# bioinfo-ut/PhenotypeSeeker

Measured on AMD Instinct MI355X. Metric: k-mer x sample chi2 cells/sec, higher is better.
Workload: dtype u64 popcount + f64; 1 GPU; synthetic 256 x 5.0-Mbp FASTA, binary phenotype, k=13; n_samples=256, k=13, rows_per_gpu=22950458, words_per_row_stored=4, survivors=1736, survivors_all_slabs=1736, device= (gfx950:sramecc+:xnack-), rows_global=22950458, collectives=none

## Files before the change

### phenotypeseeker_amd/csrc/assoc_scan.hip

```cpp
#include "chi2_launch.h"

namespace {

__device__ __forceinline__ double chi2_exact(double A, double B, double C, double D)
{
    const double w_pheno = A + B, wo_pheno = C + D, w_kmer = A + C, wo_kmer = B + D;
    const double total = w_pheno + wo_pheno;
    const double e0 = (w_pheno * w_kmer) / total, e1 = (w_pheno * wo_kmer) / total;
    const double e2 = (wo_pheno * w_kmer) / total, e3 = (wo_pheno * wo_kmer) / total;
    double stat = 0.0, d;
    d = A - e0; stat += (d * d) / e0;
    d = B - e1; stat += (d * d) / e1;
    d = C - e2; stat += (d * d) / e2;
    d = D - e3; stat += (d * d) / e3;
    return stat;
}

__device__ __forceinline__ bool chi2_keep(const ScanCuts &K, double A, double B, double C, double D, double &stat, double &p, bool valid = true)
{
    stat = chi2_exact(A, B, C, D);
    p = exp(-0.5 * stat);
    return valid && ((K.omit_B && p < K.pcut) || (p < K.pcut_bonf));
}

// ... 331 lines not shown
        b += stride;
    }
    publish_segment_once(X.s.sink);
}

template <int CPR>
__global__ __launch_bounds__(CX_IDX_THREADS) void chi2_scan_kernel_cx_side_idx(const CxSideIdxArgs X)
{
    const ScanCuts &K = X.s.cut;
    const ScanSink &S = X.s.sink;
    stamp_scan_start(S);
    if (blockIdx.x == 0) publish_unowned_segments(S);
    const int lane = threadIdx.x & 63;
    const uint64_t e0 = X.run_len[0], e1 = e0 + X.run_len[1], e2 = e1 + X.run_len[2], T = e2 + X.run_len[3];
    const uint32_t seg = blockIdx.x & (SC_NSEG - 1);
    for (uint64_t t0 = (uint64_t)blockIdx.x * CX_IDX_THREADS; t0 < T; t0 += (uint64_t)gridDim.x * CX_IDX_THREADS) {
        const uint64_t t = t0 + threadIdx.x;
        const bool live = t < T;
        uint32_t a = 0, c = 0, row = 0;
        if (live) {
            const uint64_t pos = t < e0 ? X.run_begin[0] + t : t < e1 ? X.run_begin[1] + (t - e0) : t < e2 ? X.run_begin[2] + (t - e1) : X.run_begin[3] + (t - e2);
            const uint64_t j = X.idx[pos];
            u32x4 x[CPR];
#pragma unroll
            for (int g = 0; g < CPR; g++) x[g] = PSK_CX_SIDE_NT ? __builtin_nontemporal_load(&X.s.ov[j * CPR + g]) : X.s.ov[j * CPR + g];
            row = X.s.ov_row[j];
#pragma unroll
            for (int g = 0; g < CPR; g++) {
                const uint64_t xa = ((uint64_t)x[g].y << 32) | x[g].x, xb = ((uint64_t)x[g].w << 32) | x[g].z;
                a += __popcll(xa & X.s.m1[2 * g]) + __popcll(xb & X.s.m1[2 * g + 1]);
                c += __popcll(xa & X.s.m0[2 * g]) + __popcll(xb & X.s.m0[2 * g + 1]);
            }
        }
        const int n_w = (int)(a + c);
        const int n_wo = (K.n1 - (int)a) + (K.n0 - (int)c);
        const bool freq_ok = live && !(n_w < K.min_samples || n_wo < 2 || n_w > K.max_samples);
        const double A = (double)a, B = (double)(K.n1 - (int)a), C = (double)c, D = (double)(K.n0 - (int)c);
        double stat = 0.0, p = 1.0;
        bool keep = false;
        if (freq_ok && chi2_pretest(A, B, C, D, K.thr)) keep = chi2_keep(K, A, B, C, D, stat, p);
        const uint64_t keepers = __ballot(keep);
        if (keepers) {
            uint32_t base = 0;
            if (lane == 0) base = atomicAdd(&S.counter[seg * SC_CNT_STRIDE], (uint32_t)__popcll(keepers));
            base = __builtin_amdgcn_readfirstlane(base);
            if (keep) {
                const uint32_t idx = base + (uint32_t)__popcll(keepers & ((1ull << lane) - 1ull));
                chi2_store(S, (uint64_t)seg * S.seg_cap + (idx < S.seg_cap ? idx : S.seg_cap - 1), row, stat, p, n_w);
            }
        }
    }
    publish_segment_once(S);
}

__global__ __launch_bounds__(SC_FIN_THREADS) void chi2w_finalize_kernel(const ScanArgs P)
{
    __shared__ uint32_t scan_lds[SC_FIN_THREADS / 64];
    __shared__ uint32_t s_out;
    __shared__ double2 s_tab[SC_FIN_BLK * 128];
    const uint32_t seg = blockIdx.x;
    const uint32_t c = P.sink.counter[seg * SC_CNT_STRIDE];
    const uint64_t base = (uint64_t)seg * P.sink.seg_cap;
    if (threadIdx.x == 0) s_out = 0;
    __syncthreads();
    for (uint32_t s0 = 0; s0 < c; s0 += SC_FIN_THREADS) {
        const uint32_t i = s0 + threadIdx.x;
        const bool valid = i < c;
// ... 96 lines not shown
```

### phenotypeseeker_amd/csrc/chi2_driver.hip

```cpp
#include "chi2_launch.h"

#include <cmath>
#include <sched.h>

namespace {

int pick_chi2_mode(psk_ctx *ctx, bool weighted, double pcut, double pcut_bonf, int omit_B, int *mode)
{
    double expect = pcut_bonf;
    if (omit_B && pcut > expect) expect = pcut;
    *mode = weighted ? 1 : ctx->dense_hint >= 0 ? (ctx->dense_hint ? 2 : 0) : expect > 1e-3 ? 2 : 0;
    return weighted ? PSK_OK : env_choice(ctx, "PSK_CHI2_MODE", {0, 2}, mode);
}

uint64_t cx_side_grid_cap(const psk_ctx *ctx) { return (uint64_t)(ctx->n_cu > 0 ? ctx->n_cu : 256) * (ctx->grid_mult ? ctx->grid_mult : PSK_CX_SIDE_GRID_MULT); }
uint64_t cx_pc_grid_cap(const psk_ctx *ctx) { return (uint64_t)(ctx->n_cu > 0 ? ctx->n_cu : 256) * (ctx->grid_mult ? ctx->grid_mult : PSK_CX_PC_GRID_MULT); }

int run_chi2(psk_ctx *ctx, const Chi2Launch &L, int reps, double *ms_total, double *ms_each = nullptr)
{
    *ms_total = 0;
    for (int r = 0; r < reps; r++) {
        launch_chi2_any(ctx, L, {ctx->ev0, ctx->ev1});
        PSK_HIP(ctx, hipGetLastError());
        PSK_HIP(ctx, hipStreamSynchronize(ctx->stream));
// ... 100 lines not shown
    CL.form = Chi2Form::Dense;
    ctx->last_form = (int)CL.form;
    PSK_TRY(pick_chi2_mode(ctx, L.weighted, a.cut.pcut, a.cut.pcut_bonf, a.cut.omit_B, &CL.mode));
    CL.grid = sh.grid;
    return setup_results(ctx, a, CL.grid, group_lanes(a), sh.unroll, set, sh.threads);
}

int chi2_scan_launch(psk_ctx *ctx, const int8_t *pheno, const double *weights, int min_samples, int max_samples,
                     double pvalue_cutoff, int omit_B, uint64_t n_kmers_global, bool keep_results)
{
    if (!ctx) return PSK_EINVAL;
    if (ctx->n_in_flight >= 2) return psk_fail(ctx, PSK_ESTATE, "two scans are in flight (psk_scan_end first)");
    if (!ctx->have_presence) return psk_fail(ctx, PSK_ESTATE, "no presence matrix (psk_build_presence first)");
    if (!pheno) return psk_fail(ctx, PSK_EINVAL, "null phenotype vector");
    if (n_kmers_global == 0) n_kmers_global = ctx->n_kmers ? ctx->n_kmers : 1;
    int wait_by_stamps = 1;
    PSK_TRY(env_choice(ctx, "PSK_SCAN_WAIT", {0, 1}, &wait_by_stamps));
    PSK_HIP(ctx, hipSetDevice(ctx->device));
    const int N = ctx->n_samples, wpr = mask_words(ctx);
    const size_t n_mask = 2 * (size_t)wpr, n_w = 2 * (size_t)wpr * 64;
    const size_t stage_bytes = (n_mask + n_w) * 8;
    int set = 0;
    PSK_TRY(pick_result_set(ctx, &set, keep_results));
    if (2 * stage_bytes > ctx->scan_pinned_cap) {
        if (ctx->n_in_flight) PSK_HIP(ctx, hipStreamSynchronize(ctx->stream));
        if (ctx->scan_pinned) (void)hipHostFree(ctx->scan_pinned);
        ctx->scan_pinned = nullptr;
        ctx->scan_pinned_cap = 0;
        PSK_HIP(ctx, hipHostMalloc(&ctx->scan_pinned, 2 * stage_bytes, hipHostMallocDefault));
        ctx->scan_pinned_cap = 2 * stage_bytes;
    }
    uint64_t *m1 = reinterpret_cast<uint64_t *>(static_cast<uint8_t *>(ctx->scan_pinned) + set * stage_bytes), *m0 = m1 + wpr;
// ... 22 lines not shown
    ctx->last.min_samples = min_samples;
    ctx->last.max_samples = max_samples;
    ctx->last.pvalue_cutoff = pvalue_cutoff;
    ctx->last.omit_B = omit_B ? 1 : 0;
    ctx->last.n_kmers_global = n_kmers_global;
    ctx->last.n1 = n1; ctx->last.n0 = n0; ctx->last.W1 = W1; ctx->last.W0 = W0;
    Chi2Launch CL;
    PSK_TRY(fill_chi2_args(ctx, CL, set, true));
    ctx->last_scan_kind = 1;
    if (ctx->n_kmers) {
        ScanSlot &sl = ctx->slot[set];
        const bool stamped = wait_by_stamps == 1 && !weights && !ctx->exports_async;
        launch_chi2_any(ctx, CL, stamped ? TimedBy{} : TimedBy{sl.ev0, sl.ev1});
        PSK_HIP(ctx, hipGetLastError());
        sl.stamped = stamped;
        sl.in_flight = true;
        ctx->n_in_flight++;
    } else {
        ctx->n_pass = 0;
        ctx->seg_counts.assign(SC_NSEG, 0);
        ctx->res_set = set;
        ctx->results_valid = true;
    }
    return PSK_OK;
}

int rescan(psk_ctx *ctx, int reps, double *mean_ms, double *ms_each)
{
    if (!ctx) return PSK_EINVAL;
    if (ctx->n_in_flight) return psk_fail(ctx, PSK_ESTATE, "a scan is in flight (psk_scan_end first)");
    if (!ctx->have_presence || !ctx->last.valid || ctx->last_scan_kind != 1)
        return psk_fail(ctx, PSK_ESTATE, "no chi2 scan to repeat");
    if (reps < 1) return psk_fail(ctx, PSK_EINVAL, "reps must be >= 1");
    PSK_HIP(ctx, hipSetDevice(ctx->device));
    int set = 0;
    PSK_TRY(pick_result_set(ctx, &set));
    Chi2Launch CL;
    PSK_TRY(fill_chi2_args(ctx, CL, set, false));
    double ms = 0;
    PSK_TRY(run_chi2(ctx, CL, reps, &ms, ms_each));
    ctx->last_scan_ms = ms / reps;
    PSK_TRY(fetch_counts(ctx, set));
    if (mean_ms) *mean_ms = ms / reps;
    return PSK_OK;
}

int wait_stamps(psk_ctx *ctx, int set)
{
    using clk = std::chrono::steady_clock;
    constexpr auto QUERY_EVERY = std::chrono::microseconds(20), YIELD_AFTER = std::chrono::microseconds(50);
    constexpr auto WAIT_LIMIT = std::chrono::seconds(30);
    const volatile uint64_t *counts = scan_stamp_words(ctx, set), *clocks = counts + STAMP_NSEG;
    const uint32_t seq = (uint32_t)ctx->slot[set].seq;
    int nc = 0, nk = 0;
    auto all_here = [&] {
        nc = stamp_counts_missing(counts, seq, nc);
        if (nc == STAMP_NSEG) nk = stamp_clocks_missing(clocks, seq, nk);
        return nc == STAMP_NSEG && nk == STAMP_CLOCKS;
    };
    if (!all_here()) {
        const clk::time_point t0 = clk::now();
        clk::time_point next_query = t0 + QUERY_EVERY;
        for (;;) {
            __builtin_ia32_pause();
            if (all_here()) break;
            const clk::time_point now = clk::now();
            if (now >= next_query) {
                const hipError_t e = hipStreamQuery(ctx->stream);
                if (e == hipSuccess) {
                    if (all_here()) break;
                    return psk_fail(ctx, PSK_ESTATE, "scan ended without publishing (segment %d of scan %u)", nc < STAMP_NSEG ? nc : nk, seq);
                }
                if (e != hipErrorNotReady) return psk_fail(ctx, PSK_EHIP, "hipStreamQuery failed while scan %u was awaited: %s", seq, hipGetErrorString(e));
                (void)hipGetLastError();
                if (now - t0 > WAIT_LIMIT) return psk_fail(ctx, PSK_ESTATE, "scan %u has not published its counts after 30 s", seq);
                next_query = clk::now() + QUERY_EVERY;
            }
            if (now - t0 > YIELD_AFTER) sched_yield();
        }
    }
    ctx->last_scan_ms = (double)stamp_scan_ticks(clocks) / ctx->wall_clock_khz;
    return PSK_OK;
}

}

extern "C" int psk_chi2_scan_begin(psk_ctx *ctx, const int8_t *pheno, const double *weights, int min_samples,
                                   int max_samples, double pvalue_cutoff, int omit_B, uint64_t n_kmers_global)
{
    return chi2_scan_launch(ctx, pheno, weights, min_samples, max_samples, pvalue_cutoff, omit_B, n_kmers_global, true);
}

extern "C" int psk_scan_end(psk_ctx *ctx, uint64_t *n_pass)
{
    if (!ctx) return PSK_EINVAL;
    if (ctx->n_in_flight) {
        PSK_HIP(ctx, hipSetDevice(ctx->device));
        int set = ctx->slot[0].in_flight ? 0 : 1;
        if (ctx->slot[0].in_flight && ctx->slot[1].in_flight && ctx->slot[1].seq < ctx->slot[0].seq) set = 1;
        ScanSlot &sl = ctx->slot[set];
        if (sl.stamped) {
            const int rc = wait_stamps(ctx, set);
            sl.in_flight = false;
            ctx->n_in_flight--;
            PSK_TRY(rc);
        } else {
            PSK_HIP(ctx, hipEventSynchronize(sl.ev1));
            sl.in_flight = false;
            ctx->n_in_flight--;
            float ms = 0;
            PSK_HIP(ctx, hipEventElapsedTime(&ms, sl.ev0, sl.ev1));
            ctx->last_scan_ms = ms;
        }
        PSK_TRY(fetch_counts(ctx, set));
        ctx->dense_hint = ctx->n_pass * 1000 > ctx->n_kmers ? 1 : 0;
    }
    if (n_pass) *n_pass = ctx->n_pass;
    return PSK_OK;
}

extern "C" int psk_chi2_scan(psk_ctx *ctx, const int8_t *pheno, const double *weights, int min_samples,
                             int max_samples, double pvalue_cutoff, int omit_B, uint64_t n_kmers_global,
                             uint64_t *n_pass)
{
    if (ctx && ctx->n_in_flight) return psk_fail(ctx, PSK_ESTATE, "a scan is in flight (psk_scan_end first)");
    PSK_TRY(chi2_scan_launch(ctx, pheno, weights, min_samples, max_samples, pvalue_cutoff, omit_B, n_kmers_global, false));
    return psk_scan_end(ctx, n_pass);
}

// ... 94 lines not shown
```

### phenotypeseeker_amd/csrc/psk_internal.h

```cpp
#pragma once
#include <hip/hip_runtime.h>

#include <cstdarg>
#include <cstdint>
#include <cstdio>
#include <cstdlib>
#include <cstring>
#include <chrono>
#include <functional>
#include <initializer_list>
#include <string>
#include <thread>
#include <utility>
#include <vector>

#include "../../include/psk.h"
#include "chi2_plan.h"

struct DevBuf {
    void *p = nullptr;
    size_t cap = 0;
    bool borrowed = false;
    template <class T> T *as() const { return reinterpret_cast<T *>(p); }
};
// ... 62 lines not shown
    double *res_stat, *res_p, *res_mx, *res_my;
    int32_t *res_nw;
    uint32_t *counter;
    uint32_t *final_counts;
    uint64_t *host_counts;
    uint32_t seg_cap;
    uint32_t seq;
};

struct ScanSlot {
    DevBuf res;
    ScanSink sink = {};
    bool sink_valid = false;
    hipEvent_t ev0 = nullptr, ev1 = nullptr;
    bool stamped = false;
    hipEvent_t ev_ended = nullptr;
    hipEvent_t ev_export = nullptr;
    bool export_pending = false;
    bool in_flight = false;
    uint64_t seq = 0;
    uint64_t seg_cap = 0;
};

struct psk_ctx {
    int device = 0;
    hipStream_t stream = nullptr;
    hipEvent_t ev0 = nullptr, ev1 = nullptr;
    ScanSlot slot[2];
    int res_set = 0;
    bool results_valid = false;
// ... 56 lines not shown
    bool cx_valid = false;
    uint64_t cx_n_ov = 0;
    bool cx_last_plan = false, cx_last_skipped = false, cx_last_filtered = false;
    uint64_t cx_last_rows_feasible = 0;
    uint32_t cx_last_class_mask = 0;
    int last_form = -1;
    CxPlan cx_plan;

    DevBuf mask1, phe, res_count, res_sorted;
    DevBuf lut;
    bool lut_valid = false;
    bool lut6_valid = false;
    uint64_t n_pass = 0;
    uint64_t res_seg_cap = 0;
    std::vector<uint32_t> seg_counts;
    int last_scan_kind = 0;
    int dense_hint = -1;
    double last_scan_ms = 0;
    ScanParams last;

    void *comm = nullptr;
};

int psk_fail(psk_ctx *ctx, int code, const char *fmt, ...);
std::string psk_error_text(psk_ctx *ctx);
void psk_set_error_text(psk_ctx *ctx, const std::string &text);
void psk_forget_lane_slices(psk_ctx *ctx);

#define PSK_HIP(ctx, call)                                                                            \
    do {                                                                                              \
// ... 172 lines not shown
```

### phenotypeseeker_amd/csrc/scan_common.h

```cpp
#pragma once
#include "dev_utils.h"
#include "psk_internal.h"
#include "chi2_plan.h"
#include "scan_stamps.h"

#include <hip/hip_ext.h>
#include <type_traits>

#ifndef PSK_SC_UNROLL
#define PSK_SC_UNROLL 4
#endif
#ifndef PSK_SC_GRID_MULT
#define PSK_SC_GRID_MULT 16
#endif
#ifndef PSK_SC_NT
#define PSK_SC_NT 1
#endif
constexpr int SC_THREADS = 256;
#ifndef PSK_LUT_THREADS
#define PSK_LUT_THREADS 1024
#endif
constexpr int SC_LUT_THREADS = PSK_LUT_THREADS;
constexpr size_t SC_LUT_MAX_BYTES = 132 * 1024;
constexpr int SC_UNROLL = PSK_SC_UNROLL;
// ... 32 lines not shown
    const uint32_t seg = blockIdx.x & (SC_NSEG - 1);
    const uint32_t idx = atomicAdd(&S.counter[seg * SC_CNT_STRIDE], 1u);
    return (uint64_t)seg * S.seg_cap + (idx < S.seg_cap ? idx : S.seg_cap - 1);
}

__device__ __forceinline__ void append_candidate(const ScanSink &S, uint64_t row, int n_w)
{
    const uint64_t idx = reserve_slot(S);
    S.res_row[idx] = row;
    S.res_nw[idx] = n_w;
}

__device__ __forceinline__ void stamp_store(uint64_t *p, uint64_t v) { __hip_atomic_store(p, v, __ATOMIC_RELAXED, __HIP_MEMORY_SCOPE_SYSTEM); }
__device__ __forceinline__ void stamp_clock(const ScanSink &S, int slot) { stamp_store(S.host_counts + STAMP_NSEG + slot, stamp_clock_word(S.seq, (uint64_t)wall_clock64())); }
__device__ __forceinline__ void stamp_count(const ScanSink &S, uint32_t seg, uint32_t c) { stamp_store(S.host_counts + seg, stamp_count_word(S.seq, c)); }
__device__ __forceinline__ void stamp_segment(const ScanSink &S, uint32_t seg, uint32_t c)
{
    stamp_clock(S, (int)seg);
    stamp_count(S, seg, c);
}
__device__ __forceinline__ void stamp_scan_start(const ScanSink &S)
{
    if (blockIdx.x == 0 && threadIdx.x == 0) stamp_clock(S, STAMP_START);
}

__device__ __forceinline__ void publish_segment(const ScanSink &S)
{
    __syncthreads();
    if (threadIdx.x != 0) return;
    const uint32_t seg = blockIdx.x & (SC_NSEG - 1);
    const uint32_t n_blocks = (gridDim.x - seg + SC_NSEG - 1) / SC_NSEG;
    uint32_t *slot = &S.counter[seg * SC_CNT_STRIDE];
    if (atomicAdd(slot + 1, 1u) == n_blocks - 1) {
        const uint32_t c = atomicExch(slot, 0u);
// ... 9 lines not shown
    if (threadIdx.x != 0) return;
    const uint32_t seg = blockIdx.x & (SC_NSEG - 1);
    const uint32_t n_blocks = (gridDim.x - seg + SC_NSEG - 1) / SC_NSEG;
    unsigned long long *slot = reinterpret_cast<unsigned long long *>(&S.counter[seg * SC_CNT_STRIDE]);
    const unsigned long long old = atomicAdd(slot, 1ull << 32);
    if ((uint32_t)(old >> 32) == n_blocks - 1) {
        const uint32_t c = (uint32_t)old;
        *slot = 0ull;
        S.final_counts[seg] = c;
        stamp_segment(S, seg, c);
    }
}

__device__ __forceinline__ void publish_unowned_segments(const ScanSink &S)
{
    for (uint32_t seg = gridDim.x + threadIdx.x; seg < (uint32_t)SC_NSEG; seg += blockDim.x) {
        S.final_counts[seg] = 0;
        stamp_segment(S, seg, 0);
    }
}

int mask_words(const psk_ctx *ctx);
int group_lanes(const ScanArgs &a);
uint64_t scan_grid_cap(const psk_ctx *ctx);
dim3 scan_grid(const psk_ctx *ctx, uint64_t M, int G, int unroll, bool lut = false);
uint64_t result_seg_cap(dim3 grid, uint64_t rows_per_block);
int bind_results(psk_ctx *ctx, ScanSink &s, uint64_t seg_cap, int set);
int setup_results_rows(psk_ctx *ctx, ScanSink &s, dim3 grid, uint64_t rows_per_block, int set);
int setup_results(psk_ctx *ctx, ScanArgs &a, dim3 grid, int G, int unroll, int set, int threads = SC_THREADS);
int pick_result_set(psk_ctx *ctx, int *set_out, bool keep_results = false);
int fetch_counts(psk_ctx *ctx, int set);
const volatile uint64_t *scan_stamp_words(const psk_ctx *ctx, int set);
struct ScanShape {
    dim3 grid;
    int unroll, threads;
};
int setup_table_scan(psk_ctx *ctx, ScanArgs &a, const double *tab, int nm, double s0, double s1, double s2, bool build, ScanShape *sh);

constexpr int sc_rpw(int G) { return G == 0 ? 128 : 64 / G; }
constexpr int sc_lanes(int G) { return G == 0 ? 1 : G; }
template <bool HALF>
__device__ __forceinline__ const u32x4 *sc_row_ptr(const ScanArgs &P, uint64_t r)
{
    if (HALF) return reinterpret_cast<const u32x4 *>(reinterpret_cast<const uint2 *>(P.bits) + r);
    return P.bits + r * (uint64_t)P.cpr;
}
template <bool HALF>
// ... 301 lines not shown
```

### phenotypeseeker_amd/csrc/scan_results.hip

```cpp
#include "scan_common.h"

#include <algorithm>
#include <numeric>

int mask_words(const psk_ctx *ctx) { return (ctx->wpr + 1) & ~1; }

int group_lanes(const ScanArgs &a)
{
    if (a.half) return 0;
    int G = 1;
    while (G < a.cpr && G < 64) G <<= 1;
    return G;
}

uint64_t result_seg_cap(dim3 grid, uint64_t rows_per_block) { return result_seg_cap((uint64_t)grid.x, rows_per_block); }

int bind_results(psk_ctx *ctx, ScanSink &s, uint64_t seg_cap, int set)
{
    if (seg_cap >= (1ull << 32)) return psk_fail(ctx, PSK_ERANGE, "result segment too large");
    ScanSlot &sl = ctx->slot[set];
    if (!sl.sink_valid || sl.sink.seg_cap != (uint32_t)seg_cap) {
        sl.sink_valid = false;
        const uint64_t cap = seg_cap * SC_NSEG;
        DevBuf &rb = sl.res;
        PSK_TRY(dev_reserve(ctx, rb, cap * 44 + 64));
        uint8_t *b = rb.as<uint8_t>();
        ScanSink &a = sl.sink;
        a.res_row = reinterpret_cast<uint64_t *>(b);
        a.res_stat = reinterpret_cast<double *>(b + cap * 8);
        a.res_p = reinterpret_cast<double *>(b + cap * 16);
        a.res_mx = reinterpret_cast<double *>(b + cap * 24);
        a.res_my = reinterpret_cast<double *>(b + cap * 32);
        a.res_nw = reinterpret_cast<int32_t *>(b + cap * 40);
        if (!ctx->res_count.p) {
            PSK_TRY(dev_reserve(ctx, ctx->res_count, (SC_NSEG * SC_CNT_STRIDE + 2 * SC_NSEG) * 4));
            PSK_HIP(ctx, hipMemsetAsync(ctx->res_count.p, 0, (SC_NSEG * SC_CNT_STRIDE + 2 * SC_NSEG) * 4, ctx->stream));
        }
        if (!ctx->cnt_pinned) {
            void *blk = nullptr, *hc = nullptr;
            PSK_HIP(ctx, hipHostMalloc(&blk, 2 * STAMP_SET_WORDS * 8, hipHostMallocCoherent));
            memset(blk, 0, 2 * STAMP_SET_WORDS * 8);
            if (hipHostGetDevicePointer(&hc, blk, 0) != hipSuccess) {
                (void)hipHostFree(blk);
                return psk_fail(ctx, PSK_EHIP, "hipHostGetDevicePointer failed for the scans' stamp block");
            }
            int khz = 0;
            if (hipDeviceGetAttribute(&khz, hipDeviceAttributeWallClockRate, ctx->device) != hipSuccess || khz <= 0) {
                (void)hipHostFree(blk);
                return psk_fail(ctx, PSK_EHIP, "the device reports no wall clock rate");
            }
            ctx->wall_clock_khz = khz;
            ctx->cnt_pinned = blk;
            ctx->cnt_pinned_dev = static_cast<uint64_t *>(hc);
        }
        a.counter = ctx->res_count.as<uint32_t>();
        a.final_counts = a.counter + SC_NSEG * SC_CNT_STRIDE + set * SC_NSEG;
        a.host_counts = ctx->cnt_pinned_dev + set * STAMP_SET_WORDS;
        a.seg_cap = (uint32_t)seg_cap;
        sl.sink_valid = true;
    }
    sl.stamped = false;
    sl.seq = ctx->scan_seq++;
    s = sl.sink;
    s.seq = (uint32_t)sl.seq;
    sl.seg_cap = seg_cap;
    if (set == ctx->res_set) ctx->results_valid = false;
    return PSK_OK;
}

const volatile uint64_t *scan_stamp_words(const psk_ctx *ctx, int set)
{
    return static_cast<const volatile uint64_t *>(ctx->cnt_pinned) + set * STAMP_SET_WORDS;
}

int setup_results_rows(psk_ctx *ctx, ScanSink &s, dim3 grid, uint64_t rows_per_block, int set)
{
    return bind_results(ctx, s, result_seg_cap(grid, rows_per_block), set);
}

int setup_results(psk_ctx *ctx, ScanArgs &a, dim3 grid, int G, int unroll, int set, int threads)
{
// ... 12 lines not shown
    ctx->seg_counts.assign(SC_NSEG, 0);
    uint64_t tot = 0;
    for (int s = 0; s < SC_NSEG; s++) {
        const uint64_t w = stamp_load(raw + s);
        if (stamp_word_seq(w) != seq)
            return psk_fail(ctx, PSK_ESTATE, "result segment %d carries the count of scan %u, not of scan %u", s, stamp_word_seq(w), seq);
        const uint32_t c = stamp_word_count(w);
        if (c > seg_cap) return psk_fail(ctx, PSK_ERANGE, "result segment %d overflowed (%u > %llu)", s, c, (unsigned long long)seg_cap);
        ctx->seg_counts[s] = c;
        tot += c;
    }
    ctx->n_pass = tot;
    ctx->res_set = set;
    ctx->res_seg_cap = seg_cap;
    ctx->results_valid = true;
    return PSK_OK;
}

uint64_t scan_grid_cap(const psk_ctx *ctx) { return (uint64_t)(ctx->n_cu > 0 ? ctx->n_cu : 256) * (ctx->grid_mult ? ctx->grid_mult : PSK_SC_GRID_MULT); }

dim3 scan_grid(const psk_ctx *ctx, uint64_t M, int G, int unroll, bool lut)
{
    if (lut) return dim3((unsigned)std::max(SC_NSEG, ctx->n_cu > 0 ? ctx->n_cu : 256));
    const uint64_t rpw = sc_rpw(G);
    const uint64_t steps = (M + rpw - 1) / rpw;
    const uint64_t waves = (steps + unroll - 1) / unroll;
    uint64_t blocks = (waves + SC_THREADS / 64 - 1) / (SC_THREADS / 64);
    const uint64_t cap = scan_grid_cap(ctx);
    if (blocks > cap) blocks = cap;
    if (blocks < SC_NSEG) blocks = SC_NSEG;
// ... 40 lines not shown
}

}

extern "C" int psk_get_results(psk_ctx *ctx, uint64_t *row_idx, uint64_t *words, double *stat, double *p,
                               double *mean_x, double *mean_y, int32_t *n_with, uint64_t cap)
{
    if (!ctx) return PSK_EINVAL;
    if (!ctx->last_scan_kind) return psk_fail(ctx, PSK_ESTATE, "no scan has been run");
    if (!ctx->results_valid) return psk_fail(ctx, PSK_ESTATE, "no ended scan whose results are still held (psk_scan_end first)");
    const uint64_t n = ctx->n_pass;
    if (cap < n) return psk_fail(ctx, PSK_ERANGE, "buffer too small: %llu < %llu", (unsigned long long)cap,
                                 (unsigned long long)n);
    if (n == 0) return PSK_OK;
    PSK_HIP(ctx, hipSetDevice(ctx->device));
    {
        std::vector<uint64_t> offs(SC_NSEG);
        uint64_t acc = 0;
        for (int sgm = 0; sgm < SC_NSEG; sgm++) { offs[sgm] = acc; acc += ctx->seg_counts[sgm]; }
        PSK_TRY(dev_reserve(ctx, ctx->res_sorted, n * 52 + 128 + SC_NSEG * 12));
        uint8_t *aux = ctx->res_sorted.as<uint8_t>() + ((n * 52 + 63) & ~63ull);
        uint32_t *d_cnt = reinterpret_cast<uint32_t *>(aux + SC_NSEG * 8);
        PSK_HIP(ctx, hipMemcpyAsync(aux, offs.data(), SC_NSEG * 8, hipMemcpyHostToDevice, ctx->stream));
        PSK_HIP(ctx, hipMemcpyAsync(d_cnt, ctx->seg_counts.data(), SC_NSEG * 4, hipMemcpyHostToDevice, ctx->stream));
        pack_segments_kernel<<<SC_NSEG, 256, 0, ctx->stream>>>(ctx->slot[ctx->res_set].res.as<uint8_t>(), ctx->res_seg_cap * SC_NSEG,
                                                             (uint32_t)ctx->res_seg_cap, d_cnt,
                                                             reinterpret_cast<const uint64_t *>(aux),
                                                             ctx->res_sorted.as<uint8_t>(), n,
                                                             ctx->union_words.as<uint64_t>(),
                                                             reinterpret_cast<uint64_t *>(ctx->res_sorted.as<uint8_t>() + ((n * 44 + 7) & ~7ull)));
        PSK_HIP(ctx, hipGetLastError());
        PSK_HIP(ctx, hipStreamSynchronize(ctx->stream));
    }
    const uint64_t c = n;
    const uint8_t *b = ctx->res_sorted.as<uint8_t>();
    std::vector<uint64_t> rows(n);
    std::vector<double> st(n), pv(n), mx(n), my(n);
    std::vector<int32_t> nw(n);
    PSK_HIP(ctx, hipMemcpy(rows.data(), b, n * 8, hipMemcpyDeviceToHost));
// ... 61 lines not shown
        rec[2] = f64s[2 * cap + in0 + i];
        rec[3] = f64s[3 * cap + in0 + i];
        rec[4] = f64s[4 * cap + in0 + i];
        rec[5] = (uint64_t)(int64_t)nw[in0 + i];
        for (int w = 0; w < wpr; w++) rec[6 + w] = bits[r * (uint64_t)wpr + w];
    }
}

extern "C" int psk_export_survivors(psk_ctx *ctx, void *device_dst, uint64_t cap_records, uint64_t *n_records)
{
    if (!ctx) return PSK_EINVAL;
    if (!ctx->last_scan_kind) return psk_fail(ctx, PSK_ESTATE, "no scan has been run");
    if (!ctx->results_valid) return psk_fail(ctx, PSK_ESTATE, "no ended scan whose results are still held (psk_scan_end first)");
    if (!device_dst || cap_records < 1) return psk_fail(ctx, PSK_EINVAL, "bad destination");
    PSK_HIP(ctx, hipSetDevice(ctx->device));
    if (n_records) *n_records = ctx->n_pass;
    export_records_kernel<<<SC_NSEG, SC_NSEG, 0, ctx->stream>>>(
        ctx->slot[ctx->res_set].res.as<uint8_t>(), ctx->res_seg_cap * SC_NSEG, (uint32_t)ctx->res_seg_cap,
        ctx->res_count.as<uint32_t>() + SC_NSEG * SC_CNT_STRIDE + ctx->res_set * SC_NSEG, ctx->union_words.as<uint64_t>(), ctx->bits.as<uint64_t>(),
        ctx->wpr, static_cast<uint64_t *>(device_dst),
        cap_records);
    PSK_HIP(ctx, hipGetLastError());
    PSK_HIP(ctx, hipStreamSynchronize(ctx->stream));
    return PSK_OK;
}

extern "C" int psk_export_survivors_async(psk_ctx *ctx, void *device_dst, uint64_t cap_records, void *stream)
{
    if (!ctx) return PSK_EINVAL;
    if (!ctx->last_scan_kind) return psk_fail(ctx, PSK_ESTATE, "no scan has been run");
    if (!ctx->results_valid) return psk_fail(ctx, PSK_ESTATE, "no ended scan whose results are still held (psk_scan_end first)");
    if (!device_dst || cap_records < 1) return psk_fail(ctx, PSK_EINVAL, "bad destination");
    PSK_HIP(ctx, hipSetDevice(ctx->device));
    hipStream_t st = static_cast<hipStream_t>(stream);
    ScanSlot &sl = ctx->slot[ctx->res_set];
    if (sl.stamped) {
        if (!sl.ev_ended) PSK_HIP(ctx, hipEventCreateWithFlags(&sl.ev_ended, hipEventDisableTiming));
        PSK_HIP(ctx, hipEventRecord(sl.ev_ended, ctx->stream));
        PSK_HIP(ctx, hipStreamWaitEvent(st, sl.ev_ended, 0));
    }
    ctx->exports_async = true;
    hipEvent_t &ev = sl.ev_export;
    if (!ev) PSK_HIP(ctx, hipEventCreateWithFlags(&ev, hipEventDisableTiming));
    export_records_kernel<<<SC_NSEG, SC_NSEG, 0, st>>>(
        ctx->slot[ctx->res_set].res.as<uint8_t>(), ctx->res_seg_cap * SC_NSEG, (uint32_t)ctx->res_seg_cap,
        ctx->res_count.as<uint32_t>() + SC_NSEG * SC_CNT_STRIDE + ctx->res_set * SC_NSEG, ctx->union_words.as<uint64_t>(), ctx->bits.as<uint64_t>(),
        ctx->wpr, static_cast<uint64_t *>(device_dst), cap_records);
    PSK_HIP(ctx, hipGetLastError());
// ... 7 lines not shown
```

### phenotypeseeker_amd/csrc/scan_stamps.h

```cpp
#pragma once
#include <cstdint>

#ifdef __HIPCC__
#define STAMP_SHARED __host__ __device__ inline __attribute__((always_inline))
#else
#define STAMP_SHARED inline
#endif

constexpr int STAMP_NSEG = 256;
constexpr int STAMP_CLOCKS = STAMP_NSEG + 1;
constexpr int STAMP_START = STAMP_NSEG;
constexpr int STAMP_SET_WORDS = 2 * STAMP_NSEG + 8;
constexpr uint64_t STAMP_CLOCK_MASK = (1ull << 48) - 1;

STAMP_SHARED uint64_t stamp_count_word(uint32_t seq, uint32_t count) { return ((uint64_t)seq << 32) | count; }
STAMP_SHARED uint32_t stamp_word_seq(uint64_t w) { return (uint32_t)(w >> 32); }
STAMP_SHARED uint32_t stamp_word_count(uint64_t w) { return (uint32_t)w; }
STAMP_SHARED uint64_t stamp_clock_word(uint32_t seq, uint64_t clock) { return ((uint64_t)(seq & 0xffffu) << 48) | (clock & STAMP_CLOCK_MASK); }
STAMP_SHARED uint32_t stamp_clock_tag(uint64_t w) { return (uint32_t)(w >> 48); }
STAMP_SHARED uint64_t stamp_clock_value(uint64_t w) { return w & STAMP_CLOCK_MASK; }

inline uint64_t stamp_load(const volatile uint64_t *p) { return __atomic_load_n(p, __ATOMIC_RELAXED); }

inline int stamp_counts_missing(const volatile uint64_t *counts, uint32_t seq, int from = 0)
{
    int s = from;
    while (s < STAMP_NSEG && stamp_word_seq(stamp_load(counts + s)) == seq) s++;
    return s;
}
inline bool stamp_counts_ready(const volatile uint64_t *counts, uint32_t seq) { return stamp_counts_missing(counts, seq) == STAMP_NSEG; }

inline int stamp_clocks_missing(const volatile uint64_t *clocks, uint32_t seq, int from = 0)
{
    int s = from;
    while (s < STAMP_CLOCKS && stamp_clock_tag(stamp_load(clocks + s)) == (seq & 0xffffu)) s++;
    return s;
}
inline bool stamp_clocks_ready(const volatile uint64_t *clocks, uint32_t seq) { return stamp_clocks_missing(clocks, seq) == STAMP_CLOCKS; }

inline uint64_t stamp_clock_diff(uint64_t start, uint64_t end) { return (end - start) & STAMP_CLOCK_MASK; }

inline uint64_t stamp_scan_ticks(const volatile uint64_t *clocks)
{
    const uint64_t start = stamp_clock_value(stamp_load(clocks + STAMP_START));
    uint64_t most = 1;
    for (int s = 0; s < STAMP_NSEG; s++) {
        const uint64_t d = stamp_clock_diff(start, stamp_clock_value(stamp_load(clocks + s)));
        if (d < (1ull << 47) && d > most) most = d;
    }
    return most;
}
```

### phenotypeseeker_amd/csrc/ttest_scan.hip

```cpp
#include "scan_common.h"

#include <algorithm>
#include <cmath>

namespace {

__device__ double dev_betacf(double a, double b, double x)
{
    const double TINY = 1e-300, EPS = 1e-16;
    const double qab = a + b, qap = a + 1.0, qam = a - 1.0;
    double c = 1.0, d = 1.0 - qab * x / qap;
    if (fabs(d) < TINY) d = TINY;
    d = 1.0 / d;
    double h = d;
    for (int m = 1; m <= 10000; m++) {
        const int m2 = 2 * m;
        double aa = m * (b - m) * x / ((qam + m2) * (a + m2));
        d = 1.0 + aa * d; if (fabs(d) < TINY) d = TINY;
        c = 1.0 + aa / c; if (fabs(c) < TINY) c = TINY;
        d = 1.0 / d;
        h *= d * c;
        aa = -(a + m) * (qab + m) * x / ((a + m2) * (qap + m2));
        d = 1.0 + aa * d; if (fabs(d) < TINY) d = TINY;
        c = 1.0 + aa / c; if (fabs(c) < TINY) c = TINY;
// ... 482 lines not shown
    const int G = group_lanes(a);
    PSK_TRY(setup_results(ctx, a, sh.grid, G, sh.unroll, set, sh.threads));
    ctx->n_pass = 0;
    ctx->last_scan_kind = 2;
    ctx->last.valid = false;
    if (ctx->n_kmers) {
        launch_ttest(G, sh.grid, ctx->stream, {ctx->ev0, ctx->ev1}, a, T.mu, !T.unit_w);
        PSK_HIP(ctx, hipGetLastError());
        PSK_HIP(ctx, hipStreamSynchronize(ctx->stream));
        float ms = 0;
        PSK_HIP(ctx, hipEventElapsedTime(&ms, ctx->ev0, ctx->ev1));
        ctx->last_scan_ms = ms;
        PSK_TRY(fetch_counts(ctx, set));
    } else {
        ctx->seg_counts.assign(SC_NSEG, 0);
        ctx->res_set = set;
        ctx->results_valid = true;
    }
    if (n_pass) *n_pass = ctx->n_pass;
    return PSK_OK;
}
```

Before: 781000 billion cells/s.

## Publish a single scan summary ticket and skip per-segment counter atomics for small grids

```diff
diff --git a/phenotypeseeker_amd/csrc/assoc_scan.hip b/phenotypeseeker_amd/csrc/assoc_scan.hip
--- a/phenotypeseeker_amd/csrc/assoc_scan.hip
+++ b/phenotypeseeker_amd/csrc/assoc_scan.hip
@@ -369,6 +369,8 @@
     const int lane = threadIdx.x & 63;
     const uint64_t e0 = X.run_len[0], e1 = e0 + X.run_len[1], e2 = e1 + X.run_len[2], T = e2 + X.run_len[3];
     const uint32_t seg = blockIdx.x & (SC_NSEG - 1);
+    const bool sole = CX_IDX_THREADS == 64 && gridDim.x <= (uint32_t)SC_NSEG;
+    uint32_t n_own = 0;
     for (uint64_t t0 = (uint64_t)blockIdx.x * CX_IDX_THREADS; t0 < T; t0 += (uint64_t)gridDim.x * CX_IDX_THREADS) {
         const uint64_t t = t0 + threadIdx.x;
         const bool live = t < T;
@@ -396,16 +398,24 @@
         if (freq_ok && chi2_pretest(A, B, C, D, K.thr)) keep = chi2_keep(K, A, B, C, D, stat, p);
         const uint64_t keepers = __ballot(keep);
         if (keepers) {
-            uint32_t base = 0;
-            if (lane == 0) base = atomicAdd(&S.counter[seg * SC_CNT_STRIDE], (uint32_t)__popcll(keepers));
-            base = __builtin_amdgcn_readfirstlane(base);
+            uint32_t base = n_own;
+            if (sole) n_own += (uint32_t)__popcll(keepers);
+            else {
+                if (lane == 0) base = atomicAdd(&S.counter[seg * SC_CNT_STRIDE], (uint32_t)__popcll(keepers));
+                base = __builtin_amdgcn_readfirstlane(base);
+            }
             if (keep) {
                 const uint32_t idx = base + (uint32_t)__popcll(keepers & ((1ull << lane) - 1ull));
                 chi2_store(S, (uint64_t)seg * S.seg_cap + (idx < S.seg_cap ? idx : S.seg_cap - 1), row, stat, p, n_w);
             }
         }
     }
-    publish_segment_once(S);
+    if (sole) {
+        if (threadIdx.x == 0) {
+            S.final_counts[seg] = n_own;
+            stamp_segment(S, seg, n_own);
+        }
+    } else publish_segment_once(S);
 }
 
 __global__ __launch_bounds__(SC_FIN_THREADS) void chi2w_finalize_kernel(const ScanArgs P)
diff --git a/phenotypeseeker_amd/csrc/chi2_driver.hip b/phenotypeseeker_amd/csrc/chi2_driver.hip
--- a/phenotypeseeker_amd/csrc/chi2_driver.hip
+++ b/phenotypeseeker_amd/csrc/chi2_driver.hip
@@ -138,8 +138,9 @@
     if (!ctx->have_presence) return psk_fail(ctx, PSK_ESTATE, "no presence matrix (psk_build_presence first)");
     if (!pheno) return psk_fail(ctx, PSK_EINVAL, "null phenotype vector");
     if (n_kmers_global == 0) n_kmers_global = ctx->n_kmers ? ctx->n_kmers : 1;
-    int wait_by_stamps = 1;
+    int wait_by_stamps = 1, end_by_summary = 1;
     PSK_TRY(env_choice(ctx, "PSK_SCAN_WAIT", {0, 1}, &wait_by_stamps));
+    PSK_TRY(env_choice(ctx, "PSK_SCAN_SUMMARY", {0, 1}, &end_by_summary));
     PSK_HIP(ctx, hipSetDevice(ctx->device));
     const int N = ctx->n_samples, wpr = mask_words(ctx);
     const size_t n_mask = 2 * (size_t)wpr, n_w = 2 * (size_t)wpr * 64;
@@ -192,11 +193,14 @@
         launch_chi2_any(ctx, CL, stamped ? TimedBy{} : TimedBy{sl.ev0, sl.ev1});
         PSK_HIP(ctx, hipGetLastError());
         sl.stamped = stamped;
+        sl.has_summary = stamped && stamp_summary_used(CL.grid.x);
+        sl.by_summary = sl.has_summary && end_by_summary == 1;
         sl.in_flight = true;
         ctx->n_in_flight++;
     } else {
         ctx->n_pass = 0;
         ctx->seg_counts.assign(SC_NSEG, 0);
+        ctx->counts_pending = false;
         ctx->res_set = set;
         ctx->results_valid = true;
     }
@@ -223,17 +227,22 @@
     return PSK_OK;
 }
 
-int wait_stamps(psk_ctx *ctx, int set)
+}
+
+int wait_stamps(psk_ctx *ctx, int set, StampWait what)
 {
     using clk = std::chrono::steady_clock;
     constexpr auto QUERY_EVERY = std::chrono::microseconds(20), YIELD_AFTER = std::chrono::microseconds(50);
     constexpr auto WAIT_LIMIT = std::chrono::seconds(30);
-    const volatile uint64_t *counts = scan_stamp_words(ctx, set), *clocks = counts + STAMP_NSEG;
+    const volatile uint64_t *words = scan_stamp_words(ctx, set);
     const uint32_t seq = (uint32_t)ctx->slot[set].seq;
-    int nc = 0, nk = 0;
+    const bool want_summary = what == STAMP_WAIT_SUMMARY || what == STAMP_WAIT_ALL, want_counts = what != STAMP_WAIT_SUMMARY;
+    int nc = want_counts ? 0 : STAMP_NSEG;
+    int nk = what == STAMP_WAIT_SEGMENTS ? 0 : STAMP_CLOCKS;
     auto all_here = [&] {
-        nc = stamp_counts_missing(counts, seq, nc);
-        if (nc == STAMP_NSEG) nk = stamp_clocks_missing(clocks, seq, nk);
+        if (want_summary && !stamp_summary_ready(words, seq)) return false;
+        if (nc < STAMP_NSEG) nc = stamp_counts_missing(words, seq, nc);
+        if (nc == STAMP_NSEG && nk < STAMP_CLOCKS) nk = stamp_clocks_missing(words + STAMP_NSEG, seq, nk);
         return nc == STAMP_NSEG && nk == STAMP_CLOCKS;
     };
     if (!all_here()) {
@@ -247,6 +256,7 @@
                 const hipError_t e = hipStreamQuery(ctx->stream);
                 if (e == hipSuccess) {
                     if (all_here()) break;
+                    if (want_summary && !stamp_summary_ready(words, seq)) return psk_fail(ctx, PSK_ESTATE, "scan ended without publishing (summary of scan %u)", seq);
                     return psk_fail(ctx, PSK_ESTATE, "scan ended without publishing (segment %d of scan %u)", nc < STAMP_NSEG ? nc : nk, seq);
                 }
                 if (e != hipErrorNotReady) return psk_fail(ctx, PSK_EHIP, "hipStreamQuery failed while scan %u was awaited: %s", seq, hipGetErrorString(e));
@@ -257,10 +267,9 @@
             if (now - t0 > YIELD_AFTER) sched_yield();
         }
     }
-    ctx->last_scan_ms = (double)stamp_scan_ticks(clocks) / ctx->wall_clock_khz;
-    return PSK_OK;
-}
-
+    if (want_summary) ctx->last_scan_ms = (double)stamp_summary_ticks(words) / ctx->wall_clock_khz;
+    if (what == STAMP_WAIT_SEGMENTS) ctx->last_scan_ms = (double)stamp_scan_ticks(words + STAMP_NSEG) / ctx->wall_clock_khz;
+    return PSK_OK;
 }
 
 extern "C" int psk_chi2_scan_begin(psk_ctx *ctx, const int8_t *pheno, const double *weights, int min_samples,
@@ -277,11 +286,21 @@
         int set = ctx->slot[0].in_flight ? 0 : 1;
         if (ctx->slot[0].in_flight && ctx->slot[1].in_flight && ctx->slot[1].seq < ctx->slot[0].seq) set = 1;
         ScanSlot &sl = ctx->slot[set];
+        bool counts_later = false;
         if (sl.stamped) {
-            const int rc = wait_stamps(ctx, set);
+            const int rc = wait_stamps(ctx, set, sl.by_summary ? STAMP_WAIT_SUMMARY : sl.has_summary ? STAMP_WAIT_ALL : STAMP_WAIT_SEGMENTS);
             sl.in_flight = false;
             ctx->n_in_flight--;
             PSK_TRY(rc);
+            if (sl.by_summary) {
+                const volatile uint64_t *words = scan_stamp_words(ctx, set);
+                const uint64_t hi = stamp_load(words + STAMP_SUM_HI);
+                if (stamp_sum_overflow(hi)) PSK_TRY(wait_stamps(ctx, set, STAMP_WAIT_COUNTS));
+                else {
+                    hold_results_unread(ctx, set, stamp_sum_n_pass(stamp_load(words + STAMP_SUM_LO), hi));
+                    counts_later = true;
+                }
+            }
         } else {
             PSK_HIP(ctx, hipEventSynchronize(sl.ev1));
             sl.in_flight = false;
@@ -290,7 +309,7 @@
             PSK_HIP(ctx, hipEventElapsedTime(&ms, sl.ev0, sl.ev1));
             ctx->last_scan_ms = ms;
         }
-        PSK_TRY(fetch_counts(ctx, set));
+        if (!counts_later) PSK_TRY(fetch_counts(ctx, set));
         ctx->dense_hint = ctx->n_pass * 1000 > ctx->n_kmers ? 1 : 0;
     }
     if (n_pass) *n_pass = ctx->n_pass;
diff --git a/phenotypeseeker_amd/csrc/psk_internal.h b/phenotypeseeker_amd/csrc/psk_internal.h
--- a/phenotypeseeker_amd/csrc/psk_internal.h
+++ b/phenotypeseeker_amd/csrc/psk_internal.h
@@ -100,6 +100,8 @@
     bool sink_valid = false;
     hipEvent_t ev0 = nullptr, ev1 = nullptr;
     bool stamped = false;
+    bool has_summary = false;
+    bool by_summary = false;
     hipEvent_t ev_ended = nullptr;
     hipEvent_t ev_export = nullptr;
     bool export_pending = false;
@@ -186,6 +188,7 @@
     uint64_t n_pass = 0;
     uint64_t res_seg_cap = 0;
     std::vector<uint32_t> seg_counts;
+    bool counts_pending = false;
     int last_scan_kind = 0;
     int dense_hint = -1;
     double last_scan_ms = 0;
diff --git a/phenotypeseeker_amd/csrc/scan_common.h b/phenotypeseeker_amd/csrc/scan_common.h
--- a/phenotypeseeker_amd/csrc/scan_common.h
+++ b/phenotypeseeker_amd/csrc/scan_common.h
@@ -70,10 +70,30 @@
 __device__ __forceinline__ void stamp_store(uint64_t *p, uint64_t v) { __hip_atomic_store(p, v, __ATOMIC_RELAXED, __HIP_MEMORY_SCOPE_SYSTEM); }
 __device__ __forceinline__ void stamp_clock(const ScanSink &S, int slot) { stamp_store(S.host_counts + STAMP_NSEG + slot, stamp_clock_word(S.seq, (uint64_t)wall_clock64())); }
 __device__ __forceinline__ void stamp_count(const ScanSink &S, uint32_t seg, uint32_t c) { stamp_store(S.host_counts + seg, stamp_count_word(S.seq, c)); }
+constexpr int SC_TICKET_OFFSET = SC_NSEG * SC_CNT_STRIDE + 2 * SC_NSEG;
+constexpr int SC_COUNTER_WORDS = SC_TICKET_OFFSET + SC_CNT_STRIDE;
+static_assert(SC_TICKET_OFFSET % SC_CNT_STRIDE == 0, "the ticket line starts a 128-byte line");
+__device__ __forceinline__ void publish_summary(const ScanSink &S, uint32_t c)
+{
+    unsigned long long *line = reinterpret_cast<unsigned long long *>(S.counter + SC_TICKET_OFFSET);
+    const uint64_t add = stamp_ticket_addend(c, S.seg_cap);
+    const uint64_t before = atomicAdd(line, (unsigned long long)add);
+    if (!stamp_ticket_is_last(before, stamp_ticket_publishers(gridDim.x))) return;
+    __hip_atomic_store(line, 0ull, __ATOMIC_RELAXED, __HIP_MEMORY_SCOPE_AGENT);
+    const uint64_t after = before + add;
+    stamp_store(S.host_counts + STAMP_SUM_END, stamp_clock_word(S.seq, (uint64_t)wall_clock64()));
+    stamp_store(S.host_counts + STAMP_SUM_LO, stamp_sum_lo_word(S.seq, stamp_ticket_total(after)));
+    stamp_store(S.host_counts + STAMP_SUM_HI, stamp_sum_hi_word(S.seq, stamp_ticket_total(after), stamp_ticket_overflow(after)));
+}
 __device__ __forceinline__ void stamp_segment(const ScanSink &S, uint32_t seg, uint32_t c)
 {
-    stamp_clock(S, (int)seg);
-    stamp_count(S, seg, c);
+    if (stamp_summary_used(gridDim.x)) {
+        stamp_count(S, seg, c);
+        publish_summary(S, c);
+    } else {
+        stamp_clock(S, (int)seg);
+        stamp_count(S, seg, c);
+    }
 }
 __device__ __forceinline__ void stamp_scan_start(const ScanSink &S)
 {
@@ -113,9 +133,11 @@
 
 __device__ __forceinline__ void publish_unowned_segments(const ScanSink &S)
 {
+    const bool clocks = !stamp_summary_used(gridDim.x);
     for (uint32_t seg = gridDim.x + threadIdx.x; seg < (uint32_t)SC_NSEG; seg += blockDim.x) {
         S.final_counts[seg] = 0;
-        stamp_segment(S, seg, 0);
+        if (clocks) stamp_clock(S, (int)seg);
+        stamp_count(S, seg, 0);
     }
 }
 
@@ -129,7 +151,16 @@
 int setup_results(psk_ctx *ctx, ScanArgs &a, dim3 grid, int G, int unroll, int set, int threads = SC_THREADS);
 int pick_result_set(psk_ctx *ctx, int *set_out, bool keep_results = false);
 int fetch_counts(psk_ctx *ctx, int set);
+void hold_results_unread(psk_ctx *ctx, int set, uint64_t n_pass);
+int held_seg_counts(psk_ctx *ctx, const std::vector<uint32_t> **counts);
 const volatile uint64_t *scan_stamp_words(const psk_ctx *ctx, int set);
+enum StampWait {
+    STAMP_WAIT_SUMMARY,
+    STAMP_WAIT_COUNTS,
+    STAMP_WAIT_ALL,
+    STAMP_WAIT_SEGMENTS,
+};
+int wait_stamps(psk_ctx *ctx, int set, StampWait what);
 struct ScanShape {
     dim3 grid;
     int unroll, threads;
diff --git a/phenotypeseeker_amd/csrc/scan_results.hip b/phenotypeseeker_amd/csrc/scan_results.hip
--- a/phenotypeseeker_amd/csrc/scan_results.hip
+++ b/phenotypeseeker_amd/csrc/scan_results.hip
@@ -33,8 +33,8 @@
         a.res_my = reinterpret_cast<double *>(b + cap * 32);
         a.res_nw = reinterpret_cast<int32_t *>(b + cap * 40);
         if (!ctx->res_count.p) {
-            PSK_TRY(dev_reserve(ctx, ctx->res_count, (SC_NSEG * SC_CNT_STRIDE + 2 * SC_NSEG) * 4));
-            PSK_HIP(ctx, hipMemsetAsync(ctx->res_count.p, 0, (SC_NSEG * SC_CNT_STRIDE + 2 * SC_NSEG) * 4, ctx->stream));
+            PSK_TRY(dev_reserve(ctx, ctx->res_count, SC_COUNTER_WORDS * 4));
+            PSK_HIP(ctx, hipMemsetAsync(ctx->res_count.p, 0, SC_COUNTER_WORDS * 4, ctx->stream));
         }
         if (!ctx->cnt_pinned) {
             void *blk = nullptr, *hc = nullptr;
@@ -64,7 +64,10 @@
     s = sl.sink;
     s.seq = (uint32_t)sl.seq;
     sl.seg_cap = seg_cap;
-    if (set == ctx->res_set) ctx->results_valid = false;
+    if (set == ctx->res_set) {
+        ctx->results_valid = false;
+        ctx->counts_pending = false;
+    }
     return PSK_OK;
 }
 
@@ -107,6 +110,33 @@
     ctx->res_set = set;
     ctx->res_seg_cap = seg_cap;
     ctx->results_valid = true;
+    ctx->counts_pending = false;
+    return PSK_OK;
+}
+
+void hold_results_unread(psk_ctx *ctx, int set, uint64_t n_pass)
+{
+    ctx->n_pass = n_pass;
+    ctx->res_set = set;
+    ctx->res_seg_cap = ctx->slot[set].seg_cap;
+    ctx->results_valid = true;
+    ctx->counts_pending = true;
+}
+
+int held_seg_counts(psk_ctx *ctx, const std::vector<uint32_t> **counts)
+{
+    if (ctx->counts_pending) {
+        const uint64_t n_summary = ctx->n_pass;
+        const int set = ctx->res_set;
+        PSK_TRY(wait_stamps(ctx, set, STAMP_WAIT_COUNTS));
+        PSK_TRY(fetch_counts(ctx, set));
+        if (ctx->n_pass != n_summary) {
+            ctx->results_valid = false;
+            return psk_fail(ctx, PSK_ESTATE, "the segments of scan %u hold %llu survivors, its summary said %llu", (uint32_t)ctx->slot[set].seq,
+                            (unsigned long long)ctx->n_pass, (unsigned long long)n_summary);
+        }
+    }
+    if (counts) *counts = &ctx->seg_counts;
     return PSK_OK;
 }
 
@@ -177,15 +207,17 @@
                                  (unsigned long long)n);
     if (n == 0) return PSK_OK;
     PSK_HIP(ctx, hipSetDevice(ctx->device));
+    const std::vector<uint32_t> *seg_counts = nullptr;
+    PSK_TRY(held_seg_counts(ctx, &seg_counts));
     {
         std::vector<uint64_t> offs(SC_NSEG);
         uint64_t acc = 0;
-        for (int sgm = 0; sgm < SC_NSEG; sgm++) { offs[sgm] = acc; acc += ctx->seg_counts[sgm]; }
+        for (int sgm = 0; sgm < SC_NSEG; sgm++) { offs[sgm] = acc; acc += (*seg_counts)[sgm]; }
         PSK_TRY(dev_reserve(ctx, ctx->res_sorted, n * 52 + 128 + SC_NSEG * 12));
         uint8_t *aux = ctx->res_sorted.as<uint8_t>() + ((n * 52 + 63) & ~63ull);
         uint32_t *d_cnt = reinterpret_cast<uint32_t *>(aux + SC_NSEG * 8);
         PSK_HIP(ctx, hipMemcpyAsync(aux, offs.data(), SC_NSEG * 8, hipMemcpyHostToDevice, ctx->stream));
-        PSK_HIP(ctx, hipMemcpyAsync(d_cnt, ctx->seg_counts.data(), SC_NSEG * 4, hipMemcpyHostToDevice, ctx->stream));
+        PSK_HIP(ctx, hipMemcpyAsync(d_cnt, seg_counts->data(), SC_NSEG * 4, hipMemcpyHostToDevice, ctx->stream));
         pack_segments_kernel<<<SC_NSEG, 256, 0, ctx->stream>>>(ctx->slot[ctx->res_set].res.as<uint8_t>(), ctx->res_seg_cap * SC_NSEG,
                                                              (uint32_t)ctx->res_seg_cap, d_cnt,
                                                              reinterpret_cast<const uint64_t *>(aux),
@@ -277,6 +309,7 @@
     if (!ctx->results_valid) return psk_fail(ctx, PSK_ESTATE, "no ended scan whose results are still held (psk_scan_end first)");
     if (!device_dst || cap_records < 1) return psk_fail(ctx, PSK_EINVAL, "bad destination");
     PSK_HIP(ctx, hipSetDevice(ctx->device));
+    PSK_TRY(held_seg_counts(ctx, nullptr));
     if (n_records) *n_records = ctx->n_pass;
     export_records_kernel<<<SC_NSEG, SC_NSEG, 0, ctx->stream>>>(
         ctx->slot[ctx->res_set].res.as<uint8_t>(), ctx->res_seg_cap * SC_NSEG, (uint32_t)ctx->res_seg_cap,
@@ -295,6 +328,7 @@
     if (!ctx->results_valid) return psk_fail(ctx, PSK_ESTATE, "no ended scan whose results are still held (psk_scan_end first)");
     if (!device_dst || cap_records < 1) return psk_fail(ctx, PSK_EINVAL, "bad destination");
     PSK_HIP(ctx, hipSetDevice(ctx->device));
+    PSK_TRY(held_seg_counts(ctx, nullptr));
     hipStream_t st = static_cast<hipStream_t>(stream);
     ScanSlot &sl = ctx->slot[ctx->res_set];
     if (sl.stamped) {
diff --git a/phenotypeseeker_amd/csrc/scan_stamps.h b/phenotypeseeker_amd/csrc/scan_stamps.h
--- a/phenotypeseeker_amd/csrc/scan_stamps.h
+++ b/phenotypeseeker_amd/csrc/scan_stamps.h
@@ -20,6 +20,34 @@
 STAMP_SHARED uint32_t stamp_clock_tag(uint64_t w) { return (uint32_t)(w >> 48); }
 STAMP_SHARED uint64_t stamp_clock_value(uint64_t w) { return w & STAMP_CLOCK_MASK; }
 
+constexpr int STAMP_SUM_START = 2 * STAMP_NSEG;
+constexpr int STAMP_SUM_END = STAMP_SUM_START + 1;
+constexpr int STAMP_SUM_LO = STAMP_SUM_START + 2;
+constexpr int STAMP_SUM_HI = STAMP_SUM_START + 3;
+static_assert(STAMP_SUM_HI < STAMP_SET_WORDS && STAMP_SUM_START % 8 == 0, "the summary shares the start clock's 64-byte line");
+constexpr uint64_t STAMP_NPASS_MAX = (1ull << 40) - 1;
+constexpr uint32_t STAMP_SUM_OVERFLOW = 1u << 31;
+
+STAMP_SHARED uint64_t stamp_sum_lo_word(uint32_t seq, uint64_t n_pass) { return stamp_count_word(seq, (uint32_t)n_pass); }
+STAMP_SHARED uint64_t stamp_sum_hi_word(uint32_t seq, uint64_t n_pass, bool overflow)
+{
+    return stamp_count_word(seq, (uint32_t)((n_pass & STAMP_NPASS_MAX) >> 32) | (overflow ? STAMP_SUM_OVERFLOW : 0u));
+}
+STAMP_SHARED uint64_t stamp_sum_n_pass(uint64_t lo, uint64_t hi) { return ((uint64_t)(stamp_word_count(hi) & 0xffu) << 32) | stamp_word_count(lo); }
+STAMP_SHARED bool stamp_sum_overflow(uint64_t hi) { return (stamp_word_count(hi) & STAMP_SUM_OVERFLOW) != 0; }
+
+constexpr uint32_t STAMP_SUMMARY_MAX_GRID = 64;
+STAMP_SHARED bool stamp_summary_used(uint32_t workgroups) { return workgroups <= STAMP_SUMMARY_MAX_GRID; }
+constexpr int STAMP_TICKET_SHIFT = 40, STAMP_TICKET_OVF_SHIFT = 52;
+STAMP_SHARED uint32_t stamp_ticket_publishers(uint32_t workgroups) { return workgroups < (uint32_t)STAMP_NSEG ? workgroups : (uint32_t)STAMP_NSEG; }
+STAMP_SHARED uint64_t stamp_ticket_addend(uint32_t c, uint32_t seg_cap)
+{
+    return (1ull << STAMP_TICKET_SHIFT) | (uint64_t)c | (c > seg_cap ? 1ull << STAMP_TICKET_OVF_SHIFT : 0ull);
+}
+STAMP_SHARED bool stamp_ticket_is_last(uint64_t before, uint32_t publishers) { return (uint32_t)((before >> STAMP_TICKET_SHIFT) & 0xfffu) == publishers - 1; }
+STAMP_SHARED uint64_t stamp_ticket_total(uint64_t after) { return after & STAMP_NPASS_MAX; }
+STAMP_SHARED bool stamp_ticket_overflow(uint64_t after) { return (after >> STAMP_TICKET_OVF_SHIFT) != 0; }
+
 inline uint64_t stamp_load(const volatile uint64_t *p) { return __atomic_load_n(p, __ATOMIC_RELAXED); }
 
 inline int stamp_counts_missing(const volatile uint64_t *counts, uint32_t seq, int from = 0)
@@ -38,6 +66,12 @@
 }
 inline bool stamp_clocks_ready(const volatile uint64_t *clocks, uint32_t seq) { return stamp_clocks_missing(clocks, seq) == STAMP_CLOCKS; }
 
+inline bool stamp_summary_ready(const volatile uint64_t *set_words, uint32_t seq)
+{
+    return stamp_word_seq(stamp_load(set_words + STAMP_SUM_HI)) == seq && stamp_word_seq(stamp_load(set_words + STAMP_SUM_LO)) == seq &&
+           stamp_clock_tag(stamp_load(set_words + STAMP_SUM_END)) == (seq & 0xffffu) && stamp_clock_tag(stamp_load(set_words + STAMP_SUM_START)) == (seq & 0xffffu);
+}
+
 inline uint64_t stamp_clock_diff(uint64_t start, uint64_t end) { return (end - start) & STAMP_CLOCK_MASK; }
 
 inline uint64_t stamp_scan_ticks(const volatile uint64_t *clocks)
@@ -50,3 +84,9 @@
     }
     return most;
 }
+
+inline uint64_t stamp_summary_ticks(const volatile uint64_t *set_words)
+{
+    const uint64_t d = stamp_clock_diff(stamp_clock_value(stamp_load(set_words + STAMP_SUM_START)), stamp_clock_value(stamp_load(set_words + STAMP_SUM_END)));
+    return d < (1ull << 47) && d > 1 ? d : 1;
+}
diff --git a/phenotypeseeker_amd/csrc/ttest_scan.hip b/phenotypeseeker_amd/csrc/ttest_scan.hip
--- a/phenotypeseeker_amd/csrc/ttest_scan.hip
+++ b/phenotypeseeker_amd/csrc/ttest_scan.hip
@@ -520,6 +520,7 @@
         PSK_TRY(fetch_counts(ctx, set));
     } else {
         ctx->seg_counts.assign(SC_NSEG, 0);
+        ctx->counts_pending = false;
         ctx->res_set = set;
         ctx->results_valid = true;
     }
```

Result: faster. 892400 billion cells/s (median of 6 runs) (+14.3%).
